# ANSSI-FR/libecc

Hardware: AMD Instinct MI355X
Metric: scalar-mults/sec (secp256r1, batch=2^20, variable base, affine out, bit-exact vs CPU) (higher is better)
Workload: dtype u32 (29-bit limbs, v_mad_u64_u32 integer MAD, u64 accumulators)

## Files before the change

### libecc_amd/csrc/ecamd_p256.h

```cpp
#pragma once
#include "ecamd_u29.h"

namespace p256 {
using namespace u29;

struct K {
	static constexpr u32 R2[9] = {0x00000c00, 0x00000000, 0x1fff0000, 0x1fdfffff, 0x1fbfffff,
				      0x1fffffff, 0x1fffffff, 0x1ffffffe, 0x00000013};
	static constexpr u32 ONE[9] = {0x00000020, 0x00000000, 0x00000000, 0x1fffc000, 0x1fffffff,
				       0x1fffffff, 0x1f7fffff, 0x03ffffff, 0x00000000};
	static constexpr u32 BM[9] = {0x1897bbfb, 0x1cdf6229, 0x018486c4, 0x01732821, 0x1dad59e0,
				      0x0abf7212, 0x1a06d110, 0x17721d20, 0x008600c3};
};

template <class T> U29_FN T constant(const u32 (&c)[9])
{
	T r;
#pragma unroll
	for (int i = 0; i < 9; i++) {
		r.l[i] = c[i];
	}
	return r;
}

typedef F<MASK + 16, (2ull << 24), 17> FX;
typedef F<MASK + 16, (6ull << 24) + 16, 96> FY;
typedef F<2ull * MASK, (4ull << 24), 56> FZ;
typedef F<MASK + 16, (4ull << 24), 49> FYsel;
struct TabEnt {
	FX X;
	FX Y;
	FZ Z;
};

struct Jac {
	FX X;
	FY Y;
	FZ Z;
};

U29_FN Fmul sqr_n(Fmul x, int n)
{
#pragma unroll 1
	for (int i = 0; i < n; i++) {
		x = weaken<Fmul>(sqr(x));
	}
	return x;
}
#define P256_MULW(a, b) weaken<Fmul>(mul(a, b))
U29_FN Fmul inv(const Fmul &x)
{
	const Fmul e2 = P256_MULW(sqr_n(x, 1), x);
	const Fmul e4 = P256_MULW(sqr_n(e2, 2), e2);
	const Fmul e8 = P256_MULW(sqr_n(e4, 4), e4);
	const Fmul e16 = P256_MULW(sqr_n(e8, 8), e8);
	const Fmul e32 = P256_MULW(sqr_n(e16, 16), e16);
	Fmul r = P256_MULW(sqr_n(e32, 32), x);
	r = P256_MULW(sqr_n(r, 128), e32);
	r = P256_MULW(sqr_n(r, 32), e32);
	r = P256_MULW(sqr_n(r, 16), e16);
	r = P256_MULW(sqr_n(r, 8), e8);
	r = P256_MULW(sqr_n(r, 4), e4);
	r = P256_MULW(sqr_n(r, 2), e2);
	r = P256_MULW(sqr_n(r, 2), x);
	return r;
}

U29_FN Jac dbl(const Jac &P)
{
	const auto delta = sqr(P.Z);
	const auto gamma = sqr(P.Y);
	const auto beta4 = mul(P.X, mul_small<4>(gamma));
	const auto t1 = sub<1, 0>(P.X, delta);
	const auto t2 = add(P.X, delta);
	const auto alpha0 = mul(t1, t2);
	const auto alpha = carry(mul_small<3>(alpha0));
	const auto a2 = sqr(alpha);
	const auto beta8 = mul_small<2>(beta4);
	const auto x3 = fold(sub<2, 1>(a2, beta8));
	const auto g4 = sqr(mul_small<2>(gamma));
	const auto g8 = mul_small<2>(g4);
	const auto t4 = sub<1, 1>(beta4, x3);
	const auto y3a = mul(alpha, t4);
	const auto y3 = carry(sub<2, 1>(y3a, g8));
	const auto z3 = mul_small<2>(mul(P.Y, P.Z));
	Jac R;
	R.X = weaken<FX>(x3);
	R.Y = weaken<FY>(y3);
	R.Z = weaken<FZ>(z3);
	return R;
}

template <class FX2, class FY2, class FZ2>
U29_FN Jac add_jac(const Jac &P, const FX2 &X2, const FY2 &Y2, const FZ2 &Z2, bool &h_is_zero)
{
	const auto z1z1 = sqr(P.Z);
	const auto z2z2 = sqr(Z2);
	const auto u1 = mul(P.X, z2z2);
	const auto u2 = mul(X2, z1z1);
	const auto s1 = mul(mul(P.Y, Z2), z2z2);
	const auto s2 = mul(mul(Y2, P.Z), z1z1);
	const auto h = carry(sub<1, 0>(u2, u1));
	const auto r = carry(sub<1, 0>(s2, s1));
	const auto hh = sqr(h);
	const auto hhh = mul(h, hh);
	const auto v = mul(u1, hh);
	const auto r2 = sqr(r);
	const auto x3 = fold(sub<2, 2>(r2, add(hhh, mul_small<2>(v))));
	const auto t5 = sub<1, 1>(v, x3);
	const auto m1 = mul(r, t5);
	const auto m2 = mul(s1, hhh);
	const auto y3 = carry(sub<1, 0>(m1, m2));
	const auto z3 = mul(mul(P.Z, Z2), h);
	h_is_zero = is_zero_mulout(z3);
	Jac R;
	R.X = weaken<FX>(x3);
	R.Y = weaken<FY>(y3);
	R.Z = weaken<FZ>(z3);
	return R;
}

typedef F<(1ull << 29) + MASK, (3ull << 24), 48> FYaff;
template <class FY2> U29_FN Jac madd(const Jac &P, const Fcanon &X2, const FY2 &Y2, bool &h_is_zero)
{
	const auto z1z1 = sqr(P.Z);
	const auto u2 = mul(X2, z1z1);
	const auto s2 = mul(mul(Y2, P.Z), z1z1);
	const auto h = carry(sub<1, 1>(u2, P.X));
	const auto r = carry(sub<3, 1>(s2, P.Y));
	const auto hh = sqr(h);
	const auto hhh = mul(h, hh);
	const auto v = mul(P.X, hh);
	const auto r2 = sqr(r);
	const auto x3 = fold(sub<2, 2>(r2, add(hhh, mul_small<2>(v))));
	const auto t5 = sub<1, 1>(v, x3);
	const auto y3 = carry(sub<1, 0>(mul(r, t5), mul(P.Y, hhh)));
	const auto z3 = mul(P.Z, h);
	h_is_zero = is_zero_mulout(z3);
	Jac R;
	R.X = weaken<FX>(x3);
	R.Y = weaken<FY>(y3);
	R.Z = weaken<FZ>(z3);
	return R;
}
U29_FN FYaff neg_aff(const Fcanon &y)
{
	F<0, 0, 0> zero;
#pragma unroll
	for (int i = 0; i < 9; i++) {
		zero.l[i] = 0;
	}
	return weaken<FYaff>(sub<1, 0>(zero, y));
}

U29_FN FYsel neg_y(const FX &y)
{
	F<0, 0, 0> zero;
#pragma unroll
	for (int i = 0; i < 9; i++) {
		zero.l[i] = 0;
	}
	return weaken<FYsel>(carry(sub<1, 1>(zero, y)));
}

typedef F<MASK + 16, (2ull << 24), 32> FXc;
typedef F<MASK + 16, (4ull << 24), 63> FYc;
typedef F<MASK + 15, (8ull << 24), 128> FR;
struct CoZ {
	FXc X;
	FYc Y;
};

template <class AX, class AY> U29_FN void dblu(const AX &x, const AY &y, CoZ &D, CoZ &P1, FZ &z)
{
	const Fcanon one = constant<Fcanon>(K::ONE);
	const auto gamma = sqr(y);
	const auto beta4 = mul(x, mul_small<4>(gamma));
	const auto t1 = sub<1, 0>(x, one);
	const auto t2 = add(x, one);
	const auto alpha = carry(mul_small<3>(mul(t1, t2)));
	const auto a2 = sqr(alpha);
	const auto x3 = fold(sub<2, 1>(a2, mul_small<2>(beta4)));
	const auto g8 = mul_small<2>(sqr(mul_small<2>(gamma)));
	const auto y3 = fold(sub<2, 2>(mul(alpha, sub<1, 1>(beta4, x3)), g8));
	D.X = weaken<FXc>(x3);
	D.Y = weaken<FYc>(y3);
	P1.X = weaken<FXc>(beta4);
	P1.Y = weaken<FYc>(carry(g8));
	z = weaken<FZ>(mul_small<2>(y));
}

U29_FN void zaddu(CoZ &P1, const CoZ &P2, CoZ &R, FR &r)
{
	const auto h = carry(sub<2, 1>(P1.X, P2.X));
	const auto c = sqr(h);
	const auto w1 = mul(P1.X, c);
	const auto w2 = mul(P2.X, c);
	const auto dy = carry(sub<2, 1>(P1.Y, P2.Y));
	const auto d = sqr(dy);
	const auto a1 = mul(P1.Y, sub<1, 0>(w1, w2));
	const auto x3 = fold(sub<2, 1>(d, add(w1, w2)));
	const auto y3 = carry(sub<1, 0>(mul(dy, sub<1, 1>(w1, x3)), a1));
	R.X = weaken<FXc>(x3);
	R.Y = weaken<FYc>(y3);
	P1.X = weaken<FXc>(w1);
	P1.Y = weaken<FYc>(a1);
	r = weaken<FR>(h);
}

struct QOrder {
	static constexpr u32 W[8] = {0xfc632551u, 0xf3b9cac2u, 0xa7179e84u, 0xbce6faadu, 0xffffffffu, 0xffffffffu, 0x00000000u, 0xffffffffu};
};
template <int KW, int WB> U29_FN int recode_odd(u32 *e, const u32 *kw, int slen)
{
	constexpr int NW = KW + 1;
	const u32 even = (kw[0] & 1u) - 1u;
	u64 c = 0;
#pragma unroll
	for (int w = 0; w < KW; w++) {
		c += (u64)kw[w] + (w < 8 ? (QOrder::W[w] & even) : 0u);
		e[w] = (u32)c;
		c >>= 32;
	}
	e[KW] = (u32)c;
	e[0] &= ~1u;
	const int nbits = (KW == 8) ? 257 : ((8 * slen > 256 ? 8 * slen : 256) + 1);
	const int t = (nbits + WB - 1) / WB;
	const int sh = 32 * NW - WB * t - 1;
	for (int s = 0; s < (sh >> 5); s++) {
#pragma unroll
		for (int w = NW - 1; w > 0; w--) {
			e[w] = e[w - 1];
		}
		e[0] = 0;
	}
	const int bs = sh & 31;
#pragma unroll
	for (int w = NW - 1; w > 0; w--) {
		e[w] = (u32)((((u64)e[w] << 32) | e[w - 1]) >> (32 - bs));
	}
	e[0] = (u32)(((u64)e[0] << 32) >> (32 - bs));
	e[NW - 1] |= 0x80000000u;
	return t;
}
template <int NW, int WB> U29_FN bool odd_digit(u32 *e, u32 &idx)
{
	constexpr u32 HALF = 1u << (WB - 1);
	const u32 win = e[NW - 1] >> (32 - WB);
#pragma unroll
	for (int w = NW - 1; w > 0; w--) {
		e[w] = (e[w] << WB) | (e[w - 1] >> (32 - WB));
	}
	e[0] <<= WB;
	const bool neg = win < HALF;
	idx = (win & (HALF - 1)) ^ (neg ? HALF - 1 : 0u);
	return neg;
}

U29_FN bool recode_odd64(u32 *e, const u32 *kw)
{
	const u32 even = (kw[0] & 1u) - 1u;
	u32 d[8];
	u32 borrow = 0;
#pragma unroll
	for (int w = 0; w < 8; w++) {
		const u64 x = (u64)kw[w] - QOrder::W[w] - borrow;
		d[w] = (u32)x;
		borrow = (u32)(x >> 63);
	}
	const u32 below = 0u - borrow;
	u64 c = borrow;
#pragma unroll
	for (int w = 0; w < 8; w++) {
		c += (u64)(d[w] ^ below);
		d[w] = ((u32)c & even) | (kw[w] & ~even);
		c >>= 32;
	}
#pragma unroll
	for (int w = 0; w < 7; w++) {
		e[w] = (d[w] >> 1) | (d[w + 1] << 31);
	}
	e[7] = (d[7] >> 1) | 0x80000000u;
	return (even & below) != 0u;
}

U29_FN TabEnt to_tab(const Jac &P)
{
	TabEnt T;
	T.X = P.X;
	T.Y = weaken<FX>(fold(P.Y));
	T.Z = P.Z;
	return T;
}

}
```

Measured before the change: 77.34 million.

## Replace Fermat field inversion with constant-time safegcd divsteps inversion

Adds a Bernstein-Yang safegcd inverse that runs 21 batches of 29 branchless divsteps on 29-bit signed limbs, applying each transition matrix to f/g and d/e. It also folds the Montgomery correction in by seeding e with R2. It becomes the default inv, replacing the roughly 255-squaring Fermat addition chain, which is kept behind a macro. Inversion runs once per scalar mult for the affine output, so the gain is limited to that share of the work. The new path adds signed 64-bit arithmetic and may raise register pressure.

```diff
diff --git a/libecc_amd/csrc/ecamd_p256.h b/libecc_amd/csrc/ecamd_p256.h
--- a/libecc_amd/csrc/ecamd_p256.h
+++ b/libecc_amd/csrc/ecamd_p256.h
@@ -39,6 +39,162 @@
 	FZ Z;
 };
 
+#ifndef P256_INV_FERMAT
+#define P256_INV_FERMAT 0
+#endif
+
+typedef int32_t i32;
+typedef int64_t i64;
+constexpr int SAFEGCD_N = 29;
+constexpr int SAFEGCD_BATCHES = 21;
+static_assert(SAFEGCD_N == W && SAFEGCD_N * SAFEGCD_BATCHES >= 590, "divstep count below the proven bound");
+struct DivMat {
+	i32 u, v, q, r;
+};
+
+U29_FN i32 divsteps29(i32 zeta, u32 f, u32 g, DivMat &t)
+{
+	u32 u = 1, v = 0, q = 0, r = 1;
+#pragma unroll
+	for (int i = 0; i < SAFEGCD_N; i++) {
+		u32 m1 = (u32)(zeta >> 31);
+		const u32 m2 = 0u - (g & 1u);
+		const u32 x = (f ^ m1) - m1, y = (u ^ m1) - m1, z = (v ^ m1) - m1;
+		g += x & m2;
+		q += y & m2;
+		r += z & m2;
+		m1 &= m2;
+		zeta = (i32)((u32)zeta ^ m1) - 1;
+		f += g & m1;
+		u += q & m1;
+		v += r & m1;
+		g >>= 1;
+		u <<= 1;
+		v <<= 1;
+	}
+	t.u = (i32)u;
+	t.v = (i32)v;
+	t.q = (i32)q;
+	t.r = (i32)r;
+	return zeta;
+}
+
+U29_FN void safegcd_update_fg(i32 *f, i32 *g, const DivMat &t)
+{
+	i64 cf = (i64)t.u * f[0] + (i64)t.v * g[0];
+	i64 cg = (i64)t.q * f[0] + (i64)t.r * g[0];
+	cf >>= W;
+	cg >>= W;
+#pragma unroll
+	for (int i = 1; i < 9; i++) {
+		cf += (i64)t.u * f[i] + (i64)t.v * g[i];
+		cg += (i64)t.q * f[i] + (i64)t.r * g[i];
+		f[i - 1] = (i32)((u32)cf & MASK);
+		g[i - 1] = (i32)((u32)cg & MASK);
+		cf >>= W;
+		cg >>= W;
+	}
+	f[8] = (i32)cf;
+	g[8] = (i32)cg;
+}
+
+U29_FN void safegcd_update_de(i32 *d, i32 *e, const DivMat &t)
+{
+	constexpr i32 pq[9] = {0, 0, 0, (i32)P256::Q3, 0, 0, (i32)P256::Q6, (i32)P256::Q7, (i32)P256::Q8};
+	const i32 sd = d[8] >> 31, se = e[8] >> 31;
+	i32 md = (t.u & sd) + (t.v & se);
+	i32 me = (t.q & sd) + (t.r & se);
+	i64 cd = (i64)t.u * d[0] + (i64)t.v * e[0];
+	i64 ce = (i64)t.q * d[0] + (i64)t.r * e[0];
+	md -= (i32)(((u32)md - (u32)cd) & MASK);
+	me -= (i32)(((u32)me - (u32)ce) & MASK);
+	cd -= md;
+	ce -= me;
+	cd >>= W;
+	ce >>= W;
+#pragma unroll
+	for (int i = 1; i < 9; i++) {
+		cd += (i64)t.u * d[i] + (i64)t.v * e[i];
+		ce += (i64)t.q * d[i] + (i64)t.r * e[i];
+		if (pq[i] != 0) {
+			cd += (i64)pq[i] * md;
+			ce += (i64)pq[i] * me;
+		}
+		d[i - 1] = (i32)((u32)cd & MASK);
+		e[i - 1] = (i32)((u32)ce & MASK);
+		cd >>= W;
+		ce >>= W;
+	}
+	d[8] = (i32)cd;
+	e[8] = (i32)ce;
+}
+
+U29_FN int safegcd_run(i32 *f, i32 *g, i32 *d, const u32 *x, const u32 *e0)
+{
+	i32 e[9];
+#pragma unroll
+	for (int i = 0; i < 9; i++) {
+		f[i] = (i32)P256::P[i];
+		g[i] = (i32)x[i];
+		d[i] = 0;
+		e[i] = (i32)e0[i];
+	}
+	i32 zeta = -1;
+	int steps = 0;
+#pragma unroll 1
+	for (int b = 0; b < SAFEGCD_BATCHES; b++) {
+		DivMat t;
+		zeta = divsteps29(zeta, (u32)f[0] | ((u32)f[1] << W), (u32)g[0] | ((u32)g[1] << W), t);
+		safegcd_update_de(d, e, t);
+		safegcd_update_fg(f, g, t);
+		steps += SAFEGCD_N;
+	}
+	return steps;
+}
+
+U29_FN Fcanon safegcd_normalize(i32 *d, i32 fsign)
+{
+	i32 add = d[8] >> 31;
+#pragma unroll
+	for (int i = 0; i < 9; i++) {
+		d[i] += (i32)P256::P[i] & add;
+	}
+	const i32 neg = fsign >> 31;
+#pragma unroll
+	for (int i = 0; i < 9; i++) {
+		d[i] = (d[i] ^ neg) - neg;
+	}
+#pragma unroll
+	for (int i = 0; i < 8; i++) {
+		d[i + 1] += d[i] >> W;
+		d[i] &= (i32)MASK;
+	}
+	add = d[8] >> 31;
+#pragma unroll
+	for (int i = 0; i < 9; i++) {
+		d[i] += (i32)P256::P[i] & add;
+	}
+#pragma unroll
+	for (int i = 0; i < 8; i++) {
+		d[i + 1] += d[i] >> W;
+		d[i] &= (i32)MASK;
+	}
+	Fcanon r;
+#pragma unroll
+	for (int i = 0; i < 9; i++) {
+		r.l[i] = (u32)d[i];
+	}
+	return r;
+}
+
+U29_FN Fmul inv_safegcd(const Fmul &x)
+{
+	const Fcanon xc = canonical(x);
+	i32 f[9], g[9], d[9];
+	safegcd_run(f, g, d, xc.l, K::R2);
+	return weaken<Fmul>(safegcd_normalize(d, f[8]));
+}
+
 U29_FN Fmul sqr_n(Fmul x, int n)
 {
 #pragma unroll 1
@@ -48,7 +204,7 @@
 	return x;
 }
 #define P256_MULW(a, b) weaken<Fmul>(mul(a, b))
-U29_FN Fmul inv(const Fmul &x)
+U29_FN Fmul inv_fermat(const Fmul &x)
 {
 	const Fmul e2 = P256_MULW(sqr_n(x, 1), x);
 	const Fmul e4 = P256_MULW(sqr_n(e2, 2), e2);
@@ -64,6 +220,15 @@
 	r = P256_MULW(sqr_n(r, 2), e2);
 	r = P256_MULW(sqr_n(r, 2), x);
 	return r;
+}
+
+U29_FN Fmul inv(const Fmul &x)
+{
+#if P256_INV_FERMAT
+	return inv_fermat(x);
+#else
+	return inv_safegcd(x);
+#endif
 }
 
 U29_FN Jac dbl(const Jac &P)
```

Measured after the change: 78.37 million, median of 6. 1.3% higher.
